# DannielSilva/MM-VQA

Hardware: AMD Instinct MI355X
Metric: samples/sec ROCO-MLM pretrain (resnet152+transformer, bs16/GPU, 224^2, seq32) (higher is better)
Workload: dtype f32; 1 GPU; pretrain/roco_train.py MLM-only: resnet152 + transformer(4 layers, 12 heads), num_vis 5, hidden 768, vocab 30522, per-GPU batch 16, 224x224, T=32; fwd + log_softmax/NLL + bwd + grad all-reduce + Adam; dropout on, train-mode BN; random-init weights; global_batch=16, seq_len=32, parallelism=dp1

## Files before the change

### mm-vqa_amd/csrc/common.h

```cpp
#pragma once
#include <hip/hip_runtime.h>
#include <stdint.h>
#include "../../include/mmvqa.h"

typedef float f32x4 __attribute__((ext_vector_type(4)));
typedef float f32x16 __attribute__((ext_vector_type(16)));

enum { ACT_NONE = 0, ACT_RELU = 1, ACT_GELU = 2, ACT_SERF = 3, ACT_SILU = 4, ACT_SIGMOID = 5 };
enum { PRO_NONE = 0, PRO_AFFINE_RELU = 1, PRO_DZ = 2, PRO_AFFINE = 3, PRO_AFFINE_SILU = 4, PRO_SILU_GATE = 5 };
enum { EPI_PLAIN = 0, EPI_TAP_FWD = 1, EPI_TAP_BWD = 2 };
enum { KIND_FWD = 0, KIND_DGRAD = 1, KIND_WGRAD = 2 };


typedef mmvqa_gemm_desc GemmParams;
typedef mmvqa_attn_desc AttnParams;

__device__ __forceinline__ float erf_pos(float s) {
  float t = 1.0f + s * (0.0705230784f + s * (0.0422820123f + s * (0.0092705272f +
            s * (0.0001520143f + s * (0.0002765672f + s * 0.0000430638f)))));
  t = t * t; t = t * t; t = t * t; t = t * t;
  const float big = 1.0f - 1.0f / t;
  const float s2 = s * s;
  float pl = -7.5757575757e-4f;
  pl = pl * s2 + 4.6296296296e-3f;
// ... 51 lines not shown
  }
}

__device__ __forceinline__ float rng_uniform(uint32_t seed, uint32_t idx) {
  uint32_t x = idx * 0x9E3779B1u + seed;
  x ^= x >> 16; x *= 0x7feb352du;
  x ^= x >> 15; x *= 0x846ca68bu;
  x ^= x >> 16;
  x += seed * 0x85ebca6bu;
  x ^= x >> 13; x *= 0xc2b2ae35u;
  x ^= x >> 16;
  return (float)(x >> 8) * (1.0f / 16777216.0f);
}

__device__ __forceinline__ float wave_sum(float v) {
#pragma unroll
  for (int o = 32; o > 0; o >>= 1) v += __shfl_xor(v, o, 64);
  return v;
}
__device__ __forceinline__ float wave_max(float v) {
#pragma unroll
  for (int o = 32; o > 0; o >>= 1) v = fmaxf(v, __shfl_xor(v, o, 64));
  return v;
}
__device__ __forceinline__ double wave_sum_d(double v) {
#pragma unroll
  for (int o = 32; o > 0; o >>= 1) v += __shfl_xor(v, o, 64);
  return v;
}

typedef mmvqa_bn_fold BnFold;
typedef double f64x2 __attribute__((ext_vector_type(2)));

__device__ __forceinline__ void bn_fold_sums(const double* __restrict__ stat, int slots, int C, int c, double& s0,
                                             double& s1) {
  f64x2 v[MMVQA_STAT_SLOTS];
#pragma unroll
  for (int k = 0; k < MMVQA_STAT_SLOTS; ++k) {
    v[k] = f64x2{0.0, 0.0};
    if (k < slots) v[k] = *reinterpret_cast<const f64x2*>(stat + ((size_t)k * C + c) * 2);
  }
  s0 = 0.0; s1 = 0.0;
#pragma unroll
  for (int k = 0; k < MMVQA_STAT_SLOTS; ++k) { s0 += v[k][0]; s1 += v[k][1]; }
}

__device__ __forceinline__ void bn_fold_fwd(const BnFold& f, int C, int c, bool pub, float& scale, float& shift) {
  double s, ss;
  bn_fold_sums(f.stat, f.slots, C, c, s, ss);
  const double mu = s / f.count;
  double var = ss / f.count - mu * mu;
  if (var < 0.0) var = 0.0;
  const float mean = (float)mu;
  const float invstd = (float)(1.0 / sqrt(var + (double)f.eps));
  scale = f.gamma[c] * invstd;
  shift = f.beta[c] - mean * scale;
  if (pub) {
    f.out0[c] = scale; f.out1[c] = shift; f.out2[c] = mean; f.out3[c] = invstd;
    if (f.run_mean) {
      const double unb = f.count > 1.0 ? var * (f.count / (f.count - 1.0)) : var;
      f.run_mean[c] = (float)(f.keep * (double)f.run_mean[c] + (1.0 - f.keep) * mu);
      f.run_var[c] = (float)(f.keep * (double)f.run_var[c] + (1.0 - f.keep) * unb);
    }
  }
}

template <int NCH>
__device__ __forceinline__ void bn_coef_block_fwd(const float* __restrict__ s, const float* __restrict__ b, const BnFold& f,
                                                  int C, int c0, bool pub, float (*cf)[NCH]) {
  const int t = threadIdx.x;
  if (t < NCH) {
    float a = 0.f, d = 0.f;
    const int c = c0 + t;
    if (c < C) {
      if (f.stat) bn_fold_fwd(f, C, c, pub, a, d);
      else { a = s[c]; d = b[c]; }
    }
    cf[0][t] = a; cf[1][t] = d;
  }
  __syncthreads();
}

__device__ __forceinline__ void bn_fold_bwd(const BnFold& f, int C, int c, bool pub, float& P, float& Q, float& R) {
  double sg, sgx;
  bn_fold_sums(f.stat, f.slots, C, c, sg, sgx);
  const double is = (double)f.invstd[c];
  const double p = (double)f.gamma[c] * is;
  const double c1 = sg / f.count, c2 = sgx / f.count;
  P = (float)p;
  Q = (float)(-p * c2 * is);
  R = (float)(p * (c2 * is * (double)f.mean[c] - c1));
  if (pub) {
    f.out0[c] = P; f.out1[c] = Q; f.out2[c] = R;
    f.dgamma[c] += (float)sgx;
    f.dbeta[c] += (float)sg;
  }
}

template <int NCH>
__device__ __forceinline__ void bn_coef_block_bwd(const float* __restrict__ P, const float* __restrict__ Q,
                                                  const float* __restrict__ R, const BnFold& f, int C, int c0, bool pub,
                                                  float (*cf)[NCH]) {
  const int t = threadIdx.x;
  if (t < NCH) {
    float p = 0.f, q = 0.f, r = 0.f;
    const int c = c0 + t;
    if (c < C) {
      if (f.stat) bn_fold_bwd(f, C, c, pub, p, q, r);
      else { p = P[c]; q = Q[c]; r = R[c]; }
    }
    cf[0][t] = p; cf[1][t] = q; cf[2][t] = r;
  }
  __syncthreads();
}

int mmvqa_set_error(int code, const char* fmt, ...);
#define MMVQA_OK 0
#define MMVQA_ERR_ARG -1
#define MMVQA_ERR_HIP -2
#define MMVQA_ERR_STATE -3

#define HIP_CHECK_RET(expr)                                                               \
  do {                                                                                    \
    hipError_t _e = (expr);                                                               \
    if (_e != hipSuccess)                                                                 \
      return mmvqa_set_error(MMVQA_ERR_HIP, "%s failed: %s (%s:%d)", #expr,               \
                             hipGetErrorString(_e), __FILE__, __LINE__);                  \
  } while (0)

// ... 2 lines not shown
```

### mm-vqa_amd/csrc/igemm.hip

```cpp
#include <string>
#include <type_traits>
#include <vector>

#include "kernels.h"

struct FastDiv {
  uint32_t mul, shr, d;
};
struct GemmAux {
  FastDiv ohw, ow;
  int fast;
  int stagger;
  float* part;
  int ldsc;
  int pad0;
  int sk_gx, sk_gy;
  int sk_slots;
  float* sk_part;
  unsigned* sk_cnt;
  int tick;
  int xcd;
};

__device__ __forceinline__ int fdiv(int n, const FastDiv& f) {
// ... 41 lines not shown
#define TRACE_MARK(i)                                                                              \
  do {                                                                                             \
    if (g_igemm_trace && threadIdx.x == 0 && TRACE_WG < TRACE_CAP0) {                              \
      unsigned long long* t_ = g_igemm_trace + ((size_t)(blockIdx.z * gridDim.y + blockIdx.y) * gridDim.x + blockIdx.x) * 8; \
      t_[i] = __builtin_readcyclecounter();                                                        \
      if ((i) == 0) {                                                                              \
        t_[5] = (unsigned long long)__builtin_amdgcn_s_getreg(4 | (0 << 6) | (31 << 11)) |         \
                ((unsigned long long)__builtin_amdgcn_s_getreg(20 | (0 << 6) | (31 << 11)) << 32); \
        t_[6] = __builtin_amdgcn_s_memrealtime();                                                  \
      }                                                                                            \
      if ((i) == 4) t_[7] = __builtin_amdgcn_s_memrealtime();                                      \
    }                                                                                              \
  } while (0)
#define TRACE_STALL_DECL unsigned long long tr_vm = 0, tr_lgkm = 0, tr_bar = 0;
#define TRACE_STALL_FLUSH()                                                                        \
  do {                                                                                             \
    if (g_igemm_trace && threadIdx.x == 0 && TRACE_WG < TRACE_CAP1) {                              \
      unsigned long long* t_ = g_igemm_trace + (1 << 22) + ((size_t)(blockIdx.z * gridDim.y + blockIdx.y) * gridDim.x + blockIdx.x) * 8; \
      t_[0] = tr_vm; t_[1] = tr_lgkm; t_[2] = tr_bar;                                              \
    }                                                                                              \
  } while (0)
#define TRACE_EPI(i)                                                                               \
  do {                                                                                             \
    if (g_igemm_trace && threadIdx.x == 0 && TRACE_WG < TRACE_CAP1)                                \
      g_igemm_trace[(1 << 22) + ((size_t)(blockIdx.z * gridDim.y + blockIdx.y) * gridDim.x + blockIdx.x) * 8 + 4 + (i)] = __builtin_readcyclecounter(); \
  } while (0)
#else
#define TRACE_MARK(i) do {} while (0)
#define TRACE_EPI(i) do {} while (0)
#define TRACE_STALL_DECL
#define TRACE_STALL_FLUSH() do {} while (0)
#endif

template <int BM, int BN, int NT, class Src>
__device__ __forceinline__ void general_epilogue(const GemmParams& p, int m0, int n0, int tid, float* smem, int slot_seed, Src src) {
  constexpr int CH = BN / 4;
  constexpr int RP = NT / CH;
  constexpr int NPASS = BM / RP;
  const int M = p.M, N = p.N;
  const int c4 = tid % CH, rg = tid / CH;
  const int col = n0 + c4 * 4;
  const bool full = col + 3 < N;
  auto ldv = [&](const float* base, size_t off) __attribute__((always_inline)) {
    f32x4 r = {0, 0, 0, 0};
    if (full && !(off & 3)) r = ld4(base + off);
    else {
#pragma unroll
      for (int j = 0; j < 4; ++j) if (col + j < N) r[j] = base[off + j];
    }
    return r;
  };
  auto stv = [&](float* base, size_t off, f32x4 v) __attribute__((always_inline)) {
    if (full && !(off & 3)) *reinterpret_cast<f32x4*>(base + off) = v;
    else {
#pragma unroll
      for (int j = 0; j < 4; ++j) if (col + j < N) base[off + j] = v[j];
    }
  };
  {
    float* C = p.C; const int ldc = p.c_ld;
    float* Cpre = p.Cpre;
    const float* Pre = p.Pre; const int dact = p.dact, pre_ld = p.pre_ld, act = p.act;
    const float* R = p.R; const int r_ld = p.r_ld;
    const float* Mk = p.Mk; const int mk_ld = p.mk_ld, mk_mode = p.mk_mode;
    const float* Z1 = p.Z1; const float* Z2 = p.Z2; const int z1_ld = p.z1_ld, z2_ld = p.z2_ld;
    double* st1 = p.stat1; double* st2 = p.stat2; const int stat_bwd = p.stat_bwd;
    float* colsum = p.colsum;
    const float drop_p = p.drop_p; const uint32_t drop_seed = p.drop_seed;
    const float keep_scale = drop_p > 0.f ? 1.0f / (1.0f - drop_p) : 1.f;
    const bool cok = col < N;
    f32x4 bias = {0, 0, 0, 0}, mks = {1, 1, 1, 1}, mkb = {0, 0, 0, 0};
    f32x4 mu1 = {0, 0, 0, 0}, is1 = {0, 0, 0, 0}, mu2 = {0, 0, 0, 0}, is2 = {0, 0, 0, 0};
    if (cok) {
      if (p.bias) bias = ldv(p.bias, col);
      if (Mk && p.mk_s) { mks = ldv(p.mk_s, col); mkb = ldv(p.mk_b, col); }
      if (st1 && stat_bwd) { mu1 = ldv(p.mean1, col); is1 = ldv(p.invstd1, col); }
      if (st2) { mu2 = ldv(p.mean2, col); is2 = ldv(p.invstd2, col); }
    }
    f32x4 sa = {0, 0, 0, 0}, sb = {0, 0, 0, 0}, sc = {0, 0, 0, 0}, cs = {0, 0, 0, 0};
    TRACE_EPI(3);
    constexpr int UP = NPASS < 4 ? NPASS : 4;
#pragma unroll 1
    for (int ps0 = 0; ps0 < NPASS; ps0 += UP) {
      if (m0 + rg + ps0 * RP >= M || !cok) break;
      f32x4 vv[UP], pr[UP], rr[UP], mm[UP], zz[UP], zz2[UP];
      bool ok[UP];
#pragma unroll
      for (int u = 0; u < UP; ++u) {
        const int rl = rg + (ps0 + u) * RP, row = m0 + rl;
        ok[u] = row < M;
        const size_t rw = ok[u] ? (size_t)row : (size_t)m0;
        vv[u] = src(rl, c4);
        if (dact) pr[u] = ldv(Pre, rw * pre_ld + col);
        if (R) rr[u] = ldv(R, rw * r_ld + col);
        if (Mk) mm[u] = ldv(Mk, rw * mk_ld + col);
        if (st1 && stat_bwd) {
          zz[u] = ldv(Z1, rw * z1_ld + col);
          if (st2) zz2[u] = ldv(Z2, rw * z2_ld + col);
        }
      }
#pragma unroll
      for (int u = 0; u < UP; ++u) {
        if (!ok[u]) continue;
        const int row = m0 + rg + (ps0 + u) * RP;
        f32x4 v = vv[u] + bias;
        if (Cpre) stv(Cpre, (size_t)row * ldc + col, v);
        if (dact) {
#pragma unroll
          for (int j = 0; j < 4; ++j) v[j] *= act_bwd(dact, pr[u][j]);
        }
        if (act) {
#pragma unroll
          for (int j = 0; j < 4; ++j) v[j] = act_fwd(act, v[j]);
        }
        if (drop_p > 0.f) {
#pragma unroll
          for (int j = 0; j < 4; ++j) {
            const float uu = rng_uniform(drop_seed, (uint32_t)row * (uint32_t)N + (uint32_t)(col + j));
            v[j] = (uu >= drop_p) ? v[j] * keep_scale : 0.f;
          }
        }
        if (R) v += rr[u];
        if (Mk) {
          if (mk_mode == 0) {
#pragma unroll
            for (int j = 0; j < 4; ++j) v[j] = (mm[u][j] * mks[j] + mkb[j] > 0.f) ? v[j] : 0.f;
          } else {
#pragma unroll
            for (int j = 0; j < 4; ++j) v[j] *= dsilu_f(mm[u][j] * mks[j] + mkb[j]);
          }
        }
#ifndef EXP_NOSTOREC
        stv(C, (size_t)row * ldc + col, v);
#endif
        if (st1) {
          if (stat_bwd) {
#pragma unroll
            for (int j = 0; j < 4; ++j) { sa[j] += v[j]; sb[j] += v[j] * ((zz[u][j] - mu1[j]) * is1[j]); }
            if (st2) {
#pragma unroll
              for (int j = 0; j < 4; ++j) sc[j] += v[j] * ((zz2[u][j] - mu2[j]) * is2[j]);
            }
          } else {
#pragma unroll
            for (int j = 0; j < 4; ++j) { sa[j] += v[j]; sb[j] += v[j] * v[j]; }
          }
        }
        if (colsum) cs += v;
      }
    }
    TRACE_EPI(1);
    if (st1 || colsum) {
      __syncthreads();
      double* red = reinterpret_cast<double*>(smem);
      float* redf = smem + BN * 6;
      for (int i = tid; i < BN * 3; i += NT) red[i] = 0.0;
      for (int i = tid; i < BN; i += NT) redf[i] = 0.f;
      __syncthreads();
      if (cok) {
        if (st1) {
#pragma unroll
          for (int j = 0; j < 4; ++j) {
            double* d = red + (c4 * 4 + j) * 3;
            atomicAdd(d, (double)sa[j]);
            atomicAdd(d + 1, (double)sb[j]);
            if (st2) atomicAdd(d + 2, (double)sc[j]);
          }
        }
        if (colsum) {
#pragma unroll
          for (int j = 0; j < 4; ++j) atomicAdd(&redf[c4 * 4 + j], cs[j]);
        }
      }
      __syncthreads();
      TRACE_EPI(2);
      if (tid < BN && n0 + tid < N) {
        if (st1) {
          const double* d = red + tid * 3;
          const int slot = slot_seed & ((p.stat_slots > 0 ? p.stat_slots : MMVQA_STAT_SLOTS) - 1);
          double* d1 = st1 + ((size_t)slot * N + n0 + tid) * 2;
          atomicAdd(d1, d[0]);
// ... 56 lines not shown
      by = (int)(r % gy);
      bz = (int)(r / gy);
    } else {
      by = (int)(Lg % gy);
      const unsigned r = Lg / gy;
      bx = (int)(r % gx);
      bz = (int)(r / gx);
    }
  }
  const int m0 = by * BM, n0 = bx * BN;
#ifdef EXP_SAMETILE
  const int lm0 = 0, ln0 = 0;
#else
  const int lm0 = m0, ln0 = n0;
#endif

  const int kt_begin = bz * p.ktiles_per_split;
  int kt_end = kt_begin + p.ktiles_per_split;
  if (kt_end > nkt_total) kt_end = nkt_total;
  const int nkt = kt_end - kt_begin;
  const int k_begin = kt_begin * BK;

  const int OHW = p.g_OH * p.g_OW;
  const int taps = p.g_KH * p.g_KW;
  const int s = p.g_stride;

  if (!NCHW && A_ROWK && tid < MAX_TAPS) {
    int t = tid < taps ? tid : 0;
    int kh = t / p.g_KW, kw = t - kh * p.g_KW;
    int off = (KIND == KIND_FWD) ? (kh * p.g_SW + kw) * p.a_ld : -((kh / s) * p.g_SW + (kw / s)) * p.a_ld;
    taptab[tid] = off;
  }
  const int fold_C = A_ROWK ? p.g_Cs : BM;
  if (x.ldsc) {
    const BnFold& f = p.a_fold;
    const bool pub = f.publish && bx == 0 && by == 0 && bz == 0;
    if constexpr (A_ROWK) {
      for (int c = tid; c < fold_C; c += NT) {
        float k0, k1, k2 = 0.f;
        if (f.bwd) bn_fold_bwd(f, fold_C, c, pub, k0, k1, k2); else bn_fold_fwd(f, fold_C, c, pub, k0, k1);
        ctab[c] = k0; ctab[fold_C + c] = k1;
        if (f.bwd) ctab[2 * fold_C + c] = k2;
      }
      if (pub && tid == 0 && !f.bwd && f.nbt) *f.nbt += f.reps;
    } else {
      if (tid < BM) {
        const int c = lm0 + tid;
        float k0 = 1.f, k1 = 0.f, k2 = 0.f;
        if (c < p.M) { if (f.bwd) bn_fold_bwd(f, p.M, c, false, k0, k1, k2); else bn_fold_fwd(f, p.M, c, false, k0, k1); }
        ctab[tid] = k0; ctab[BM + tid] = k1; ctab[2 * BM + tid] = k2;
      }
    }
  }
  __syncthreads();

  const int a_kq = (tid % KQ) * 4;
  const int a_r0 = tid / KQ;
  int a_base[NAC];
  uint32_t a_mask[NAC];
  int a_c = 0, a_tap = 0;
  int a_pix[NAC], a_y0[NAC], a_x0[NAC];
  int a_img[NAC];
  f32x4 ac0_i = {1, 1, 1, 1}, ac1_i = {0, 0, 0, 0}, ac2_i = {0, 0, 0, 0};
  const int akm_x4 = tid % A_X4, akm_k0 = tid / A_X4;
  if constexpr (A_ROWK) {
    if (x.fast == 0) {
      int k = k_begin + a_kq;
      if (taps > 1) { a_tap = k / p.g_Cs; a_c = k - a_tap * p.g_Cs; } else { a_c = k; a_tap = (k >= p.g_Cs) ? 1 : 0; }
    }
#pragma unroll
    for (int r = 0; r < NA; ++r) {
      const int row = lm0 + a_r0 + RSTEP * r;
      a_base[r] = 0; a_mask[r] = 0; a_pix[r] = 0; a_y0[r] = -(1 << 24); a_x0[r] = -(1 << 24); a_img[r] = 0;
      if (row < p.M) {
        const int n = fdiv(row, x.ohw), rem = row - n * OHW;
        const int oy = fdiv(rem, x.ow), ox = rem - oy * p.g_OW;
        if (p.gate_hw > 0) a_img[r] = row / p.gate_hw;
        if constexpr (NCHW) {
          a_pix[r] = n; a_y0[r] = oy * s - p.g_pad; a_x0[r] = ox * s - p.g_pad;
        } else if (KIND == KIND_FWD) {
          const int y0 = oy * s - p.g_pad, x0 = ox * s - p.g_pad;
          a_base[r] = ((n * p.g_SH + y0) * p.g_SW + x0) * p.a_ld;
          uint32_t xb = 0;
          for (int kw = 0; kw < p.g_KW; ++kw) xb |= ((unsigned)(x0 + kw) < (unsigned)p.g_SW ? 1u : 0u) << kw;
          uint32_t mk = 0;
          for (int kh = 0; kh < p.g_KH; ++kh) mk |= ((unsigned)(y0 + kh) < (unsigned)p.g_SH ? xb : 0u) << (kh * p.g_KW);
// ... 2 lines not shown
          const int ty = oy + p.g_pad, tx = ox + p.g_pad;
          if (s <= 2) {
            const int sh = s - 1, sm = s - 1;
            const int qy = ty >> sh, ry = ty & sm, qx = tx >> sh, rx = tx & sm;
            a_base[r] = ((n * p.g_SH + qy) * p.g_SW + qx) * p.a_ld;
            uint32_t xb = 0;
            for (int kw = 0; kw < p.g_KW; ++kw)
              xb |= (((kw & sm) == rx && (unsigned)(qx - (kw >> sh)) < (unsigned)p.g_SW) ? 1u : 0u) << kw;
            uint32_t mk = 0;
            for (int kh = 0; kh < p.g_KH; ++kh)
              mk |= (((kh & sm) == ry && (unsigned)(qy - (kh >> sh)) < (unsigned)p.g_SH) ? xb : 0u) << (kh * p.g_KW);
            a_mask[r] = mk;
          } else {
            const int qy = ty / s, ry = ty - qy * s, qx = tx / s, rx = tx - qx * s;
            a_base[r] = ((n * p.g_SH + qy) * p.g_SW + qx) * p.a_ld;
            uint32_t mk = 0;
            for (int t = 0; t < taps; ++t) {
              const int kh = t / p.g_KW, kw = t - kh * p.g_KW;
              const int sy = qy - kh / s, sx = qx - kw / s;
              if ((kh % s) == ry && (kw % s) == rx && sy >= 0 && sy < p.g_SH && sx >= 0 && sx < p.g_SW) mk |= 1u << t;
            }
            a_mask[r] = mk;
          }
        }
      }
    }
  } else {
    const int i = lm0 + akm_x4 * 4;
#pragma unroll
    for (int r = 0; r < NA_KM; ++r) {
      a_base[r] = (k_begin + akm_k0 + A_KSTEP * r) * p.a_ld + i;
      a_mask[r] = (i < p.M) ? 1u : 0u;
    }
    if (p.a_pro != PRO_NONE && i < p.M) {
      if (x.ldsc) {
        ac0_i = *reinterpret_cast<const f32x4*>(&ctab[akm_x4 * 4]);
        ac1_i = *reinterpret_cast<const f32x4*>(&ctab[BM + akm_x4 * 4]);
        ac2_i = *reinterpret_cast<const f32x4*>(&ctab[2 * BM + akm_x4 * 4]);
      } else {
        ac0_i = ld4(p.a_c0 + i); ac1_i = ld4(p.a_c1 + i);
        if (p.a_pro == PRO_DZ) ac2_i = ld4(p.a_c2 + i);
      }
    }
  }

  const int b_kq = (tid % KQ) * 4, b_r0 = tid / KQ;
  const int bkm_x4 = tid % B_X4, bkm_k0 = tid / B_X4;
  int b_base[NBC];
  uint32_t b_ok0[NBC];
  int b_co[NBC], b_tap[NBC];
  f32x4 bc0 = {1, 1, 1, 1}, bc1 = {0, 0, 0, 0};
  int b_kh = 0, b_kw = 0, b_ci = 0;
  int b_dy[4], b_dx[4], b_cc[4];
  bool b_colvalid = true;
  if constexpr (KIND == KIND_FWD) {
#pragma unroll
    for (int r = 0; r < NB; ++r) {
      const int n = ln0 + b_r0 + RSTEP * r;
      b_ok0[r] = n < p.N;
      b_base[r] = (n < p.N ? n : 0) * p.b_ld + b_kq + k_begin;
    }
  } else if constexpr (KIND == KIND_DGRAD) {
    const int n = ln0 + bkm_x4 * 4;
    b_colvalid = n < p.N;
#pragma unroll
    for (int r = 0; r < NB_KM; ++r) {
      int k = k_begin + bkm_k0 + B_KSTEP * r;
      b_tap[r] = 0; b_co[r] = k;
      if (x.fast == 0) {
        if (taps > 1) { b_tap[r] = k / p.g_Cs; b_co[r] = k - b_tap[r] * p.g_Cs; }
        else { b_tap[r] = (k >= p.g_Cs) ? 1 : 0; }
      }
      b_base[r] = n; b_ok0[r] = 1;
    }
  } else {
// ... 9 lines not shown
      for (int j = 0; j < 4; ++j) {
        int kk = nn + j;
        int tap = kk / p.g_Cs;
        b_cc[j] = kk - tap * p.g_Cs;
        b_dy[j] = tap / p.g_KW; b_dx[j] = tap - b_dy[j] * p.g_KW;
        if (kk >= p.N) b_dy[j] = -(1 << 24);
      }
    }
#pragma unroll
    for (int r = 0; r < NB_KM; ++r) { b_base[r] = k_begin + bkm_k0 + B_KSTEP * r; b_ok0[r] = 1; }
  }

  struct Stage {
    f32x4 ra[NAC], ra2[NAC], rb[NBC], rb2[NBC];
    uint32_t a_ok, b_ok;
    f32x4 ac0, ac1, ac2;
    int tm[NAC];
    int pm[NBC], tmb[NBC];
  };

  f32x16 acc[TM][TN];
#pragma unroll
  for (int i = 0; i < TM; ++i)
#pragma unroll
    for (int j = 0; j < TN; ++j)
#pragma unroll
      for (int e = 0; e < 16; ++e) acc[i][j][e] = 0.f;

  const int adv_tap = BK / p.g_Cs, adv_c = BK - adv_tap * p.g_Cs;

  auto lds_put = [&](float* tile, int e, f32x4 v) __attribute__((always_inline)) {
    if constexpr (F16) *reinterpret_cast<f16x4*>(reinterpret_cast<_Float16*>(tile) + e) = __builtin_convertvector(v, f16x4);
    else *reinterpret_cast<f32x4*>(&tile[e]) = v;
  };

  auto run = [&](auto APRO_T, auto BPRO_T, auto FAST_T, auto LDSC_T) __attribute__((always_inline)) {
    constexpr int APRO = decltype(APRO_T)::value;
    constexpr int BPRO = decltype(BPRO_T)::value;
    constexpr int FAST = decltype(FAST_T)::value;
    constexpr bool LDSC = decltype(LDSC_T)::value;
    constexpr bool A_TWO = (APRO == PRO_DZ);
    constexpr bool A_AFF = (APRO == PRO_AFFINE_RELU || APRO == PRO_AFFINE_SILU || APRO == PRO_SILU_GATE);
    constexpr bool B_AFF = (BPRO == PRO_AFFINE_RELU || BPRO == PRO_AFFINE_SILU || BPRO == PRO_SILU_GATE);

    constexpr int NLP = 1 + NAC + NBC;
    bool lt_kvalid = false;
    int lt_toff = 0;
    int lt_kh[4], lt_kw[4], lt_c[4];
    auto load_piece = [&](Stage& S, int kt, int i) __attribute__((always_inline)) {
      if (i == 0) {
        S.a_ok = 0; S.b_ok = 0;
        if constexpr (A_ROWK && !NCHW) {
          lt_kvalid = a_tap < taps;
          lt_toff = taptab[lt_kvalid ? a_tap : 0];
          if constexpr (A_AFF || A_TWO) {
            const int cc = lt_kvalid ? a_c : 0;
            S.ac0 = ld4(p.a_c0 + cc); S.ac1 = ld4(p.a_c1 + cc);
            if constexpr (APRO == PRO_DZ) S.ac2 = ld4(p.a_c2 + cc);
          }
        }
        if constexpr (NCHW) {
          S.a_ok = S.b_ok = ~0u;
          if constexpr (A_ROWK) {
#pragma unroll
            for (int j = 0; j < 4; ++j) {
              const int kk = kt * BK + a_kq + j;
// ... 192 lines not shown
        rB = __builtin_amdgcn_make_buffer_rsrc((void*)p.B, 0, p.N * p.b_ld * 4, FLAGS);
#pragma unroll
        for (int r = 0; r < NBC; ++r) f_voffB[r] = b_ok0[r] ? b_base[r] * 4 : BIG;
      } else if constexpr (KIND == KIND_DGRAD) {
        rB = __builtin_amdgcn_make_buffer_rsrc((void*)p.B, 0, p.g_Cs * p.b_ld * 4, FLAGS);
#pragma unroll
        for (int r = 0; r < NBC; ++r)
          f_voffB[r] = b_colvalid ? ((bkm_k0 + B_KSTEP * r) * p.b_ld + b_base[r]) * 4 : BIG;
      } else if constexpr (FAST == 1) {
        rB = __builtin_amdgcn_make_buffer_rsrc((void*)p.B, 0, p.K * p.b_ld * 4, FLAGS);
#pragma unroll
        for (int r = 0; r < NBC; ++r) f_voffB[r] = b_colvalid ? (b_base[r] * p.b_ld + b_ci) * 4 : BIG;
      } else {
        f_tapw = n0 / p.g_Cs;
        const int kh = f_tapw / p.g_KW, kw = f_tapw - kh * p.g_KW;
        rB = __builtin_amdgcn_make_buffer_rsrc((void*)(p.B - (p.g_pad * p.g_SW + p.g_pad) * p.b_ld), 0, NREC, FLAGS);
        rT = __builtin_amdgcn_make_buffer_rsrc((void*)p.pixmask, 0, p.K * 4, FLAGS);
        f_runB = (kh * p.g_SW + kw) * p.b_ld * 4;
#pragma unroll
        for (int r = 0; r < NBC; ++r) {
          f_voffB[r] = b_colvalid ? (b_base[r] * p.b_ld + b_ci) * 4 : BIG;
          f_voffT[r] = b_base[r] * 4;
        }
      }
#pragma unroll
      for (int r = 0; r < NBC; ++r) f_veB[r] = f_voffB[r];
    }
    int f_ve[NAC];
#pragma unroll
    for (int r = 0; r < NAC; ++r) f_ve[r] = (FAST != 0) ? f_voffA[r] : 0;
    auto tload = [&](int voff, int soff) __attribute__((always_inline)) {
      return __builtin_amdgcn_raw_buffer_load_b32(rT, voff, soff, 0);
    };
    auto f_halo = [&](Stage& S) __attribute__((always_inline)) {
      if constexpr (FAST == 2 && KIND == KIND_WGRAD) {
#pragma unroll
        for (int r = 0; r < NBC; ++r) {
          const int t = __builtin_amdgcn_sbfe(S.pm[r], f_tapw, 1);
          S.tmb[r] = t;
          f_veB[r] = (t & f_voffB[r]) | (~t & BIG);
          S.pm[r] = tload(f_voffT[r], f_runT + 2 * BK * 4);
        }
      } else if constexpr (FAST == 2) {
#pragma unroll
        for (int r = 0; r < NAC; ++r) {
          const int t = __builtin_amdgcn_sbfe((int)a_mask[r], f_tap & 31, 1);
          S.tm[r] = t;
          f_ve[r] = (t & f_voffA[r]) | (~t & BIG);
        }
      }
    };
    auto f_scalars = [&](Stage& S) __attribute__((always_inline)) {
      if constexpr (A_ROWK) {
        const bool live = f_tap < taps;
        const int toff = (KIND == KIND_FWD) ? (f_kh * p.g_SW + f_kw) * p.a_ld
                                            : f_maxneg - ((f_kh >> f_sh) * p.g_SW + (f_kw >> f_sh)) * p.a_ld;
        f_sA = live ? (toff + f_c) * 4 : BIG;
        f_sC = live ? f_c * 4 : BIG;
        if constexpr (KIND == KIND_DGRAD) f_sB = live ? (f_c * p.b_ld + f_tap * p.b_tapstride) * 4 : BIG;
        else f_sB = f_runB;
        if constexpr ((A_AFF || A_TWO) && LDSC) {
          const float* cp = ctab + f_c + a_kq;
          S.ac0 = *reinterpret_cast<const f32x4*>(cp); S.ac1 = *reinterpret_cast<const f32x4*>(cp + fold_C);
          if constexpr (APRO == PRO_DZ) S.ac2 = *reinterpret_cast<const f32x4*>(cp + 2 * fold_C);
        } else if constexpr (A_AFF || A_TWO) {
          S.ac0 = bload(rC0, f_voffC, f_sC); S.ac1 = bload(rC1, f_voffC, f_sC);
          if constexpr (APRO == PRO_DZ) S.ac2 = bload(rC2, f_voffC, f_sC);
        }
      } else {
        f_sA = f_runA; f_sB = f_runB;
      }
    };
    auto f_chunk = [&](Stage& S, int i) __attribute__((always_inline)) {
      if (i < NAC) {
        S.ra[i] = bload(rA, f_ve[i], f_sA);
        if constexpr (A_TWO) S.ra2[i] = bload(rA2, f_ve[i], f_sA);
      } else {
        S.rb[i - NAC] = bload(rB, f_veB[i - NAC], f_sB);
      }
    };
    auto f_advance = [&]() __attribute__((always_inline)) {
#ifdef EXP_NOADVANCE
      return;
#endif
      if constexpr (A_ROWK) {
        f_c += BK;
        if (f_c >= p.g_Cs) {
          f_c = 0; ++f_tap; ++f_kw;
          if (f_kw == p.g_KW) { f_kw = 0; ++f_kh; }
        }
        f_runB += BK * 4;
      } else {
        f_runA += BK * p.a_ld * 4;
        f_runB += BK * p.b_ld * 4;
        f_runT += BK * 4;
      }
    };
    auto fload_piece = [&](Stage& S, int i) __attribute__((always_inline)) {
      if (i == 0) { f_halo(S); f_scalars(S); }
      else f_chunk(S, i - 1);
      if (i == NLP - 1) f_advance();
    };
    auto fstore_chunk = [&](Stage& S, int buf, int c) __attribute__((always_inline)) {
      float* as = As + buf * A_TILE;
      float* bs = Bs + buf * B_TILE;
// ... 27 lines not shown
        } else {
          lds_put(as, (akm_k0 + A_KSTEP * r) * LDA_KM + akm_x4 * 4, v);
        }
      } else {
        const int r = c - NAC;
        f32x4 v = S.rb[r];
        if constexpr (KIND == KIND_WGRAD && BPRO == PRO_AFFINE_RELU) {
          const f32x2 lo = __builtin_elementwise_fma(v.xy, bc0.xy, bc1.xy), hi = __builtin_elementwise_fma(v.zw, bc0.zw, bc1.zw);
          if constexpr (FAST == 2) {
            const float lim = __builtin_bit_cast(float, S.tmb[r] & 0x7f800000);
            v[0] = __builtin_amdgcn_fmed3f(lo[0], 0.f, lim); v[1] = __builtin_amdgcn_fmed3f(lo[1], 0.f, lim);
            v[2] = __builtin_amdgcn_fmed3f(hi[0], 0.f, lim); v[3] = __builtin_amdgcn_fmed3f(hi[1], 0.f, lim);
          } else {
            v[0] = fmaxf(lo[0], 0.f); v[1] = fmaxf(lo[1], 0.f); v[2] = fmaxf(hi[0], 0.f); v[3] = fmaxf(hi[1], 0.f);
          }
        }
        if constexpr (B_ROWK) {
          lds_put(bs, (b_r0 + RSTEP * r) * LDK + b_kq, v);
        } else {
          lds_put(bs, (bkm_k0 + B_KSTEP * r) * LDB_KM + bkm_x4 * 4, v);
        }
      }
    };
    auto LP = [&](Stage& S, int kt, int i) __attribute__((always_inline)) {
      if constexpr (FAST != 0) fload_piece(S, i); else load_piece(S, kt, i);
    };
    auto SC = [&](Stage& S, int buf, int kt, int c) __attribute__((always_inline)) {
      if constexpr (FAST != 0) fstore_chunk(S, buf, c); else store_chunk(S, buf, kt, c);
    };
    auto LT = [&](Stage& S, int kt) __attribute__((always_inline)) {
#pragma unroll
      for (int i = 0; i < NLP; ++i) LP(S, kt, i);
    };

    auto read_frags = [&](const float* as, const float* bs, int kg, f32x4 (&fa)[TM], f32x4 (&fb)[TN]) __attribute__((always_inline)) {
#pragma unroll
      for (int i = 0; i < TM; ++i) {
        if constexpr (A_ROWK) {
          fa[i] = *reinterpret_cast<const f32x4*>(&as[(wm0 + i * 32 + li) * LDK + kg * 8 + lh * 4]);
        } else {
#pragma unroll
          for (int j = 0; j < 4; ++j) fa[i][j] = as[(kg * 8 + lh * 4 + j) * LDA_KM + wm0 + i * 32 + li];
        }
      }
#pragma unroll
      for (int i = 0; i < TN; ++i) {
        if constexpr (B_ROWK) {
          fb[i] = *reinterpret_cast<const f32x4*>(&bs[(wn0 + i * 32 + li) * LDK + kg * 8 + lh * 4]);
        } else {
#pragma unroll
          for (int j = 0; j < 4; ++j) fb[i][j] = bs[(kg * 8 + lh * 4 + j) * LDB_KM + wn0 + i * 32 + li];
        }
      }
    };

    constexpr int NC = NAC + NBC;
    constexpr int NKG = BK / 8 / KS;

    TRACE_MARK(1);
    Stage S0, S1;
    S0.a_ok = S0.b_ok = S1.a_ok = S1.b_ok = 0;
    S0.ac0 = S1.ac0 = ac0_i; S0.ac1 = S1.ac1 = ac1_i; S0.ac2 = S1.ac2 = ac2_i;

    if constexpr (FAST == 2 && KIND == KIND_WGRAD) {
#pragma unroll
      for (int r = 0; r < NBC; ++r) { S0.pm[r] = tload(f_voffT[r], 0); S1.pm[r] = tload(f_voffT[r], BK * 4); }
    }
    if (nkt > 0) {
      LT(S0, kt_begin);
      if constexpr (PIPE) LT(S1, kt_begin + 1);
#pragma unroll
      for (int c = 0; c < NC; ++c) SC(S0, 0, kt_begin, c);
      if constexpr (FAST != 0 && PIPE && !F16) f_halo(S0);
    }
    __builtin_amdgcn_s_waitcnt(0x0F70);
    __syncthreads();
    TRACE_MARK(2);

    if constexpr (F16) {
      auto frag = [&](const float* tile, int rowk, int ldkm, int r0, int st) __attribute__((always_inline)) {
        const _Float16* t = reinterpret_cast<const _Float16*>(tile);
        if (rowk) return *reinterpret_cast<const f16x8*>(t + (r0 + li) * LDK + st * 16 + lh * 8);
        const int g = lane >> 4, q = (lane >> 2) & 3, pp = lane & 3;
        const _Float16* b = t + (st * 16 + (g >> 1) * 8 + q) * ldkm + r0 + (g & 1) * 16 + 4 * pp;
        typedef __attribute__((address_space(3))) s16x4 lds_s16x4;
        const f16x4 lo = __builtin_bit_cast(f16x4, __builtin_amdgcn_ds_read_tr16_b64_v4i16((lds_s16x4*)(b)));
        const f16x4 hi = __builtin_bit_cast(f16x4, __builtin_amdgcn_ds_read_tr16_b64_v4i16((lds_s16x4*)(b + 4 * ldkm)));
        return __builtin_shufflevector(lo, hi, 0, 1, 2, 3, 4, 5, 6, 7);
      };
      auto body16 = [&](int t, Stage& Sload, Stage& Sstore) __attribute__((always_inline)) {
        const int buf = t & 1;
        LT(Sload, kt_begin + t + (PIPE ? 2 : 1));
        const float* as = As + buf * A_TILE;
        const float* bs = Bs + buf * B_TILE;
#pragma unroll
        for (int st = 0; st < BK / 16; ++st) {
          f16x8 fa[TM], fb[TN];
#pragma unroll
          for (int i = 0; i < TM; ++i) fa[i] = frag(as, A_ROWK, LDA_KM, wm0 + i * 32, st);
#pragma unroll
          for (int i = 0; i < TN; ++i) fb[i] = frag(bs, B_ROWK, LDB_KM, wn0 + i * 32, st);
#pragma unroll
          for (int a = 0; a < TM; ++a)
// ... 188 lines not shown
      } else if (x.fast == 2) {
        if constexpr (TM * TN == 1) {
          if (p.a_pro == PRO_DZ) {
            if (p.b_pro == PRO_AFFINE_RELU) run(I2{}, I1{}, F2{}, L0{}); else run(I2{}, I0{}, F2{}, L0{});
          } else {
            if (p.b_pro == PRO_AFFINE_RELU) run(I0{}, I1{}, F2{}, L0{}); else run(I0{}, I0{}, F2{}, L0{});
          }
        }
      } else if (p.a_pro == PRO_DZ) {
        switch (p.b_pro) {
          case PRO_AFFINE_RELU: run(I2{}, I1{}, G{}, L0{}); break;
          case PRO_AFFINE_SILU: run(I2{}, I4{}, G{}, L0{}); break;
          case PRO_SILU_GATE: run(I2{}, I5{}, G{}, L0{}); break;
          default: run(I2{}, I0{}, G{}, L0{});
        }
      } else {
        switch (p.b_pro) {
          case PRO_AFFINE_RELU: run(I0{}, I1{}, G{}, L0{}); break;
          case PRO_AFFINE_SILU: run(I0{}, I4{}, G{}, L0{}); break;
          case PRO_SILU_GATE: run(I0{}, I5{}, G{}, L0{}); break;
          default: run(I0{}, I0{}, G{}, L0{});
        }
      }
    }
  }

  TRACE_MARK(3);
  TRACE_STALL_FLUSH();
  constexpr int LDC = BN + 4;
  constexpr int CH = BN / 4;
  constexpr int RP = NT / CH;
  constexpr int NPASS = BM / RP;
  float* ctile = smem;
  if (KS == 1 || ks == 0) {
    static_for<TM * TN * 16>([&](auto I) {
      constexpr int i = decltype(I)::value;
      constexpr int a = i / (TN * 16), b = (i / 16) % TN, e = i % 16;
      ctile[(wm0 + a * 32 + (e & 3) + 8 * (e >> 2) + 4 * lh) * LDC + wn0 + b * 32 + li] = acc[a][b][e];
    });
  }
  __syncthreads();
  if constexpr (KS > 1) {
    if (ks == 1) {
      static_for<TM * TN * 16>([&](auto I) {
        constexpr int i = decltype(I)::value;
        constexpr int a = i / (TN * 16), b = (i / 16) % TN, e = i % 16;
        ctile[(wm0 + a * 32 + (e & 3) + 8 * (e >> 2) + 4 * lh) * LDC + wn0 + b * 32 + li] += acc[a][b][e];
      });
    }
    __syncthreads();
  }

  TRACE_EPI(0);
  const int M = p.M, N = p.N;
  const int c4 = tid % CH, rg = tid / CH;
  const int col = n0 + c4 * 4;
  const bool full = col + 3 < N;
  auto ldv = [&](const float* base, size_t off) __attribute__((always_inline)) {
    f32x4 r = {0, 0, 0, 0};
    if (full && !(off & 3)) r = ld4(base + off);
    else {
#pragma unroll
      for (int j = 0; j < 4; ++j) if (col + j < N) r[j] = base[off + j];
    }
    return r;
  };
  auto stv = [&](float* base, size_t off, f32x4 v) __attribute__((always_inline)) {
    if (full && !(off & 3)) *reinterpret_cast<f32x4*>(base + off) = v;
    else {
#pragma unroll
      for (int j = 0; j < 4; ++j) if (col + j < N) base[off + j] = v[j];
    }
  };

  if (x.tick != 0) {
    const int n_contrib = x.sk_slots, my = bz, tile_id = by * x.sk_gx + bx;
    constexpr int Q = BM * BN / 4;
    __amdgpu_buffer_rsrc_t rP = __builtin_amdgcn_make_buffer_rsrc((void*)(x.sk_part + (size_t)tile_id * x.sk_slots * (BM * BN)), 0,
                                                                  x.sk_slots * BM * BN * 4, 0x00020000);
    typedef int i32x4 __attribute__((ext_vector_type(4)));
    for (int i = tid; i < Q; i += NT) {
      const int r = i / (BN / 4), c = i - r * (BN / 4);
      const f32x4 v = *reinterpret_cast<const f32x4*>(&ctile[r * LDC + c * 4]);
      __builtin_amdgcn_raw_buffer_store_b128(__builtin_bit_cast(i32x4, v), rP, (my * Q + i) * 16, 0, SC1_AUX);
    }
    asm volatile("s_waitcnt vmcnt(0)" ::: "memory");
// ... 85 lines not shown
    }
    flush();
    __syncthreads();
    for (int i = tid; i < NIMG * BN; i += NT) {
      const int sl = i / BN, cl = i - sl * BN;
      const float v = lacc[i];
      if (v != 0.f && n0 + cl < N) atomicAdd(&out[(size_t)(img0 + sl) * N + n0 + cl], v);
    }
    TRACE_MARK(4);
    return;
  }

  if (p.epi_mode == EPI_TAP_BWD) {
    const int act = p.act, HW = p.tap_HW, ldc = p.c_ld;
    const float inv_hw = 1.0f / (float)HW;
    const float* dv = p.tap_dv;
    float* C = p.C;
#pragma unroll 1
    for (int ps = 0; ps < NPASS; ++ps) {
      const int rl = rg + ps * RP, row = m0 + rl;
      if (row >= M || col >= N) break;
      const int img = row / HW;
      f32x4 v = *reinterpret_cast<const f32x4*>(&ctile[rl * LDC + c4 * 4]);
      const f32x4 g = ldv(dv, (size_t)img * N + col);
#pragma unroll
      for (int j = 0; j < 4; ++j) v[j] = g[j] * inv_hw * act_bwd(act, v[j]);
      stv(C, (size_t)row * ldc + col, v);
    }
    TRACE_MARK(4);
    return;
  }

  general_epilogue<BM, BN, NT>(p, m0, n0, tid, smem, (int)(blockIdx.y + blockIdx.x * 7 + blockIdx.z * 3),
                               [&](int rl, int cq) __attribute__((always_inline)) {
                                 return *reinterpret_cast<const f32x4*>(&ctile[rl * LDC + cq * 4]);
                               });
  TRACE_MARK(4);
}

constexpr int FOLD_MAX_FLOATS = 3072;
constexpr int SK_MAX = 8;

__global__ __launch_bounds__(256) void splitk_finish_kernel(const GemmParams p, const float* __restrict__ part,
                                                            int nsplit) {
  constexpr int BM = 64, BN = 64;
  __shared__ double smem_d[BN * 3 + BN / 2 + 2];
  const int tid = threadIdx.x, m0 = blockIdx.y * BM, n0 = blockIdx.x * BN;
  const int M = p.M, N = p.N;
  const size_t MN = (size_t)M * N;
  general_epilogue<BM, BN, 256>(p, m0, n0, tid, reinterpret_cast<float*>(smem_d), (int)(blockIdx.y + blockIdx.x * 7),
                                [&](int rl, int cq) __attribute__((always_inline)) {
                                  f32x4 v = {0, 0, 0, 0};
                                  const int row = m0 + rl, col = n0 + cq * 4;
                                  if (row < M && col < N) {
                                    const size_t off = (size_t)row * N + col;
                                    if (col + 3 < N && !(off & 3)) {
                                      f32x4 t[SK_MAX];
#pragma unroll
                                      for (int s = 0; s < SK_MAX; ++s)
                                        t[s] = s < nsplit ? ld4(part + s * MN + off) : f32x4{0, 0, 0, 0};
#pragma unroll
                                      for (int s = 0; s < SK_MAX; ++s) v += t[s];
                                    } else {
                                      for (int s = 0; s < nsplit; ++s)
#pragma unroll
                                        for (int j = 0; j < 4; ++j)
                                          if (col + j < N) v[j] += part[s * MN + off + j];
                                    }
                                  }
                                  return v;
                                });
}

static FastDiv make_fastdiv(int d) {
  FastDiv f;
  f.d = (uint32_t)d;
  if (d <= 1) { f.mul = 0; f.shr = 0; f.d = 1; return f; }
  int lg = 31;
  while (lg > 0 && !((uint32_t)d >> lg)) --lg;
  if (d & (d - 1)) ++lg;
  const int pw = 31 + lg;
  const uint64_t m = ((1ull << pw) + (uint64_t)d - 1) / (uint64_t)d;
  f.mul = (uint32_t)m;
// ... 329 lines not shown
```

Measured before the change: 662.8 samples/s.

## Overlap BN-fold stat loads and epilogue side loads with GEMM prologue and staging

The BN fold coefficient computation now issues its stat and parameter loads early (bn_fold_issue) and finishes the table only after the first A/B tile loads are in flight, so that global-load latency overlaps. In the plain epilogue, side-tensor loads (residual, pre-activation, mask, BN inputs) are issued before the accumulator is staged to shared memory, hiding their latency behind the LDS writes and barrier. The stat fold loop is also changed from a fixed full-slot unroll to grouped loads of four slots with a runtime loop, and the per-element stat accumulation is vectorized. This adds control complexity and register pressure in the GEMM prologue and epilogue.

```diff
diff --git a/mm-vqa_amd/csrc/common.h b/mm-vqa_amd/csrc/common.h
--- a/mm-vqa_amd/csrc/common.h
+++ b/mm-vqa_amd/csrc/common.h
@@ -107,29 +107,57 @@
 typedef mmvqa_bn_fold BnFold;
 typedef double f64x2 __attribute__((ext_vector_type(2)));
 
+#define BN_FOLD_GROUP 4
+__device__ __forceinline__ void bn_fold_group(const double* __restrict__ stat, int slots, int C, int c, int k0,
+                                              f64x2 (&v)[BN_FOLD_GROUP]) {
+#pragma unroll
+  for (int j = 0; j < BN_FOLD_GROUP; ++j) {
+    v[j] = f64x2{0.0, 0.0};
+    if (k0 + j < slots) v[j] = *reinterpret_cast<const f64x2*>(stat + ((size_t)(k0 + j) * C + c) * 2);
+  }
+}
+__device__ __forceinline__ void bn_fold_sums_from(const double* __restrict__ stat, int slots, int C, int c,
+                                                  const f64x2 (&v0)[BN_FOLD_GROUP], double& s0, double& s1) {
+  s0 = 0.0; s1 = 0.0;
+#pragma unroll
+  for (int j = 0; j < BN_FOLD_GROUP; ++j) { s0 += v0[j][0]; s1 += v0[j][1]; }
+#pragma unroll 1
+  for (int k0 = BN_FOLD_GROUP; k0 < slots; k0 += BN_FOLD_GROUP) {
+    f64x2 v[BN_FOLD_GROUP];
+    bn_fold_group(stat, slots, C, c, k0, v);
+#pragma unroll
+    for (int j = 0; j < BN_FOLD_GROUP; ++j) { s0 += v[j][0]; s1 += v[j][1]; }
+  }
+}
 __device__ __forceinline__ void bn_fold_sums(const double* __restrict__ stat, int slots, int C, int c, double& s0,
                                              double& s1) {
-  f64x2 v[MMVQA_STAT_SLOTS];
-#pragma unroll
-  for (int k = 0; k < MMVQA_STAT_SLOTS; ++k) {
-    v[k] = f64x2{0.0, 0.0};
-    if (k < slots) v[k] = *reinterpret_cast<const f64x2*>(stat + ((size_t)k * C + c) * 2);
-  }
-  s0 = 0.0; s1 = 0.0;
-#pragma unroll
-  for (int k = 0; k < MMVQA_STAT_SLOTS; ++k) { s0 += v[k][0]; s1 += v[k][1]; }
-}
-
-__device__ __forceinline__ void bn_fold_fwd(const BnFold& f, int C, int c, bool pub, float& scale, float& shift) {
+  f64x2 v0[BN_FOLD_GROUP];
+  bn_fold_group(stat, slots, C, c, 0, v0);
+  bn_fold_sums_from(stat, slots, C, c, v0, s0, s1);
+}
+
+struct BnFoldIn {
+  f64x2 v0[BN_FOLD_GROUP];
+  float g, b, m;
+};
+__device__ __forceinline__ void bn_fold_issue(const BnFold& f, bool bwd, int C, int c, BnFoldIn& in) {
+  bn_fold_group(f.stat, f.slots, C, c, 0, in.v0);
+  const float* pb = bwd ? f.invstd : f.beta;
+  const float* pm = bwd ? f.mean : f.gamma;
+  in.g = f.gamma[c]; in.b = pb[c]; in.m = pm[c];
+}
+
+__device__ __forceinline__ void bn_fold_fwd_from(const BnFold& f, int C, int c, bool pub, const BnFoldIn& in, float& scale,
+                                                 float& shift) {
   double s, ss;
-  bn_fold_sums(f.stat, f.slots, C, c, s, ss);
+  bn_fold_sums_from(f.stat, f.slots, C, c, in.v0, s, ss);
   const double mu = s / f.count;
   double var = ss / f.count - mu * mu;
   if (var < 0.0) var = 0.0;
   const float mean = (float)mu;
   const float invstd = (float)(1.0 / sqrt(var + (double)f.eps));
-  scale = f.gamma[c] * invstd;
-  shift = f.beta[c] - mean * scale;
+  scale = in.g * invstd;
+  shift = in.b - mean * scale;
   if (pub) {
     f.out0[c] = scale; f.out1[c] = shift; f.out2[c] = mean; f.out3[c] = invstd;
     if (f.run_mean) {
@@ -138,6 +166,11 @@
       f.run_var[c] = (float)(f.keep * (double)f.run_var[c] + (1.0 - f.keep) * unb);
     }
   }
+}
+__device__ __forceinline__ void bn_fold_fwd(const BnFold& f, int C, int c, bool pub, float& scale, float& shift) {
+  BnFoldIn in;
+  bn_fold_issue(f, false, C, c, in);
+  bn_fold_fwd_from(f, C, c, pub, in, scale, shift);
 }
 
 template <int NCH>
@@ -156,20 +189,26 @@
   __syncthreads();
 }
 
-__device__ __forceinline__ void bn_fold_bwd(const BnFold& f, int C, int c, bool pub, float& P, float& Q, float& R) {
+__device__ __forceinline__ void bn_fold_bwd_from(const BnFold& f, int C, int c, bool pub, const BnFoldIn& in, float& P,
+                                                 float& Q, float& R) {
   double sg, sgx;
-  bn_fold_sums(f.stat, f.slots, C, c, sg, sgx);
-  const double is = (double)f.invstd[c];
-  const double p = (double)f.gamma[c] * is;
+  bn_fold_sums_from(f.stat, f.slots, C, c, in.v0, sg, sgx);
+  const double is = (double)in.b;
+  const double p = (double)in.g * is;
   const double c1 = sg / f.count, c2 = sgx / f.count;
   P = (float)p;
   Q = (float)(-p * c2 * is);
-  R = (float)(p * (c2 * is * (double)f.mean[c] - c1));
+  R = (float)(p * (c2 * is * (double)in.m - c1));
   if (pub) {
     f.out0[c] = P; f.out1[c] = Q; f.out2[c] = R;
     f.dgamma[c] += (float)sgx;
     f.dbeta[c] += (float)sg;
   }
+}
+__device__ __forceinline__ void bn_fold_bwd(const BnFold& f, int C, int c, bool pub, float& P, float& Q, float& R) {
+  BnFoldIn in;
+  bn_fold_issue(f, true, C, c, in);
+  bn_fold_bwd_from(f, C, c, pub, in, P, Q, R);
 }
 
 template <int NCH>
diff --git a/mm-vqa_amd/csrc/igemm.hip b/mm-vqa_amd/csrc/igemm.hip
--- a/mm-vqa_amd/csrc/igemm.hip
+++ b/mm-vqa_amd/csrc/igemm.hip
@@ -97,8 +97,8 @@
 #define TRACE_STALL_FLUSH() do {} while (0)
 #endif
 
-template <int BM, int BN, int NT, class Src>
-__device__ __forceinline__ void general_epilogue(const GemmParams& p, int m0, int n0, int tid, float* smem, int slot_seed, Src src) {
+template <int BM, int BN, int NT, class Stage, class Src>
+__device__ __forceinline__ void general_epilogue(const GemmParams& p, int m0, int n0, int tid, float* smem, int slot_seed, Stage stage, Src src) {
   constexpr int CH = BN / 4;
   constexpr int RP = NT / CH;
   constexpr int NPASS = BM / RP;
@@ -143,19 +143,15 @@
       if (st2) { mu2 = ldv(p.mean2, col); is2 = ldv(p.invstd2, col); }
     }
     f32x4 sa = {0, 0, 0, 0}, sb = {0, 0, 0, 0}, sc = {0, 0, 0, 0}, cs = {0, 0, 0, 0};
-    TRACE_EPI(3);
     constexpr int UP = NPASS < 4 ? NPASS : 4;
-#pragma unroll 1
-    for (int ps0 = 0; ps0 < NPASS; ps0 += UP) {
-      if (m0 + rg + ps0 * RP >= M || !cok) break;
-      f32x4 vv[UP], pr[UP], rr[UP], mm[UP], zz[UP], zz2[UP];
-      bool ok[UP];
+    f32x4 pr[UP], rr[UP], mm[UP], zz[UP], zz2[UP];
+    bool ok[UP];
+    auto side_loads = [&](int ps0) __attribute__((always_inline)) {
 #pragma unroll
       for (int u = 0; u < UP; ++u) {
-        const int rl = rg + (ps0 + u) * RP, row = m0 + rl;
+        const int row = m0 + rg + (ps0 + u) * RP;
         ok[u] = row < M;
         const size_t rw = ok[u] ? (size_t)row : (size_t)m0;
-        vv[u] = src(rl, c4);
         if (dact) pr[u] = ldv(Pre, rw * pre_ld + col);
         if (R) rr[u] = ldv(R, rw * r_ld + col);
         if (Mk) mm[u] = ldv(Mk, rw * mk_ld + col);
@@ -164,6 +160,11 @@
           if (st2) zz2[u] = ldv(Z2, rw * z2_ld + col);
         }
       }
+    };
+    auto passes = [&](int ps0) __attribute__((always_inline)) {
+      f32x4 vv[UP];
+#pragma unroll
+      for (int u = 0; u < UP; ++u) vv[u] = src(rg + (ps0 + u) * RP, c4);
 #pragma unroll
       for (int u = 0; u < UP; ++u) {
         if (!ok[u]) continue;
@@ -199,19 +200,28 @@
         stv(C, (size_t)row * ldc + col, v);
 #endif
         if (st1) {
+          sa += v;
           if (stat_bwd) {
-#pragma unroll
-            for (int j = 0; j < 4; ++j) { sa[j] += v[j]; sb[j] += v[j] * ((zz[u][j] - mu1[j]) * is1[j]); }
-            if (st2) {
-#pragma unroll
-              for (int j = 0; j < 4; ++j) sc[j] += v[j] * ((zz2[u][j] - mu2[j]) * is2[j]);
-            }
+            sb += v * ((zz[u] - mu1) * is1);
+            if (st2) sc += v * ((zz2[u] - mu2) * is2);
           } else {
-#pragma unroll
-            for (int j = 0; j < 4; ++j) { sa[j] += v[j]; sb[j] += v[j] * v[j]; }
+            sb += v * v;
           }
         }
         if (colsum) cs += v;
+      }
+    };
+    const bool rows0 = cok && m0 + rg < M;
+    if (rows0) side_loads(0);
+    stage();
+    TRACE_EPI(3);
+    if (rows0) {
+      passes(0);
+#pragma unroll 1
+      for (int ps0 = UP; ps0 < NPASS; ps0 += UP) {
+        if (m0 + rg + ps0 * RP >= M) break;
+        side_loads(ps0);
+        passes(ps0);
       }
     }
     TRACE_EPI(1);
@@ -334,26 +344,9 @@
     taptab[tid] = off;
   }
   const int fold_C = A_ROWK ? p.g_Cs : BM;
-  if (x.ldsc) {
-    const BnFold& f = p.a_fold;
-    const bool pub = f.publish && bx == 0 && by == 0 && bz == 0;
-    if constexpr (A_ROWK) {
-      for (int c = tid; c < fold_C; c += NT) {
-        float k0, k1, k2 = 0.f;
-        if (f.bwd) bn_fold_bwd(f, fold_C, c, pub, k0, k1, k2); else bn_fold_fwd(f, fold_C, c, pub, k0, k1);
-        ctab[c] = k0; ctab[fold_C + c] = k1;
-        if (f.bwd) ctab[2 * fold_C + c] = k2;
-      }
-      if (pub && tid == 0 && !f.bwd && f.nbt) *f.nbt += f.reps;
-    } else {
-      if (tid < BM) {
-        const int c = lm0 + tid;
-        float k0 = 1.f, k1 = 0.f, k2 = 0.f;
-        if (c < p.M) { if (f.bwd) bn_fold_bwd(f, p.M, c, false, k0, k1, k2); else bn_fold_fwd(f, p.M, c, false, k0, k1); }
-        ctab[tid] = k0; ctab[BM + tid] = k1; ctab[2 * BM + tid] = k2;
-      }
-    }
-  }
+  const int fold_N = A_ROWK ? p.g_Cs : p.M;
+  const int fold_c = A_ROWK ? tid : lm0 + (tid & (BM - 1));
+  BnFoldIn fold_in;
   __syncthreads();
 
   const int a_kq = (tid % KQ) * 4;
@@ -422,15 +415,9 @@
       a_base[r] = (k_begin + akm_k0 + A_KSTEP * r) * p.a_ld + i;
       a_mask[r] = (i < p.M) ? 1u : 0u;
     }
-    if (p.a_pro != PRO_NONE && i < p.M) {
-      if (x.ldsc) {
-        ac0_i = *reinterpret_cast<const f32x4*>(&ctab[akm_x4 * 4]);
-        ac1_i = *reinterpret_cast<const f32x4*>(&ctab[BM + akm_x4 * 4]);
-        ac2_i = *reinterpret_cast<const f32x4*>(&ctab[2 * BM + akm_x4 * 4]);
-      } else {
-        ac0_i = ld4(p.a_c0 + i); ac1_i = ld4(p.a_c1 + i);
-        if (p.a_pro == PRO_DZ) ac2_i = ld4(p.a_c2 + i);
-      }
+    if (p.a_pro != PRO_NONE && i < p.M && !x.ldsc) {
+      ac0_i = ld4(p.a_c0 + i); ac1_i = ld4(p.a_c1 + i);
+      if (p.a_pro == PRO_DZ) ac2_i = ld4(p.a_c2 + i);
     }
   }
 
@@ -506,6 +493,32 @@
   auto lds_put = [&](float* tile, int e, f32x4 v) __attribute__((always_inline)) {
     if constexpr (F16) *reinterpret_cast<f16x4*>(reinterpret_cast<_Float16*>(tile) + e) = __builtin_convertvector(v, f16x4);
     else *reinterpret_cast<f32x4*>(&tile[e]) = v;
+  };
+
+  auto fold_table = [&]() __attribute__((always_inline)) {
+    const BnFold& f = p.a_fold;
+    if constexpr (A_ROWK) {
+      const bool pub = f.publish && bx == 0 && by == 0 && bz == 0;
+      if (tid < fold_C) {
+        float k0, k1, k2 = 0.f;
+        if (f.bwd) bn_fold_bwd_from(f, fold_C, tid, pub, fold_in, k0, k1, k2); else bn_fold_fwd_from(f, fold_C, tid, pub, fold_in, k0, k1);
+        ctab[tid] = k0; ctab[fold_C + tid] = k1;
+        if (f.bwd) ctab[2 * fold_C + tid] = k2;
+      }
+      for (int c = tid + NT; c < fold_C; c += NT) {
+        float k0, k1, k2 = 0.f;
+        if (f.bwd) bn_fold_bwd(f, fold_C, c, pub, k0, k1, k2); else bn_fold_fwd(f, fold_C, c, pub, k0, k1);
+        ctab[c] = k0; ctab[fold_C + c] = k1;
+        if (f.bwd) ctab[2 * fold_C + c] = k2;
+      }
+      if (pub && tid == 0 && !f.bwd && f.nbt) *f.nbt += f.reps;
+    } else {
+      if (tid < BM) {
+        float k0 = 1.f, k1 = 0.f, k2 = 0.f;
+        if (fold_c < p.M) { if (f.bwd) bn_fold_bwd_from(f, p.M, fold_c, false, fold_in, k0, k1, k2); else bn_fold_fwd_from(f, p.M, fold_c, false, fold_in, k0, k1); }
+        ctab[tid] = k0; ctab[BM + tid] = k1; ctab[2 * BM + tid] = k2;
+      }
+    }
   };
 
   auto run = [&](auto APRO_T, auto BPRO_T, auto FAST_T, auto LDSC_T) __attribute__((always_inline)) {
@@ -764,6 +777,11 @@
     auto tload = [&](int voff, int soff) __attribute__((always_inline)) {
       return __builtin_amdgcn_raw_buffer_load_b32(rT, voff, soff, 0);
     };
+    auto take_coef = [&](Stage& S, int c) __attribute__((always_inline)) {
+      const float* cp = ctab + c + a_kq;
+      S.ac0 = *reinterpret_cast<const f32x4*>(cp); S.ac1 = *reinterpret_cast<const f32x4*>(cp + fold_C);
+      if constexpr (APRO == PRO_DZ) S.ac2 = *reinterpret_cast<const f32x4*>(cp + 2 * fold_C);
+    };
     auto f_halo = [&](Stage& S) __attribute__((always_inline)) {
       if constexpr (FAST == 2 && KIND == KIND_WGRAD) {
 #pragma unroll
@@ -782,7 +800,8 @@
         }
       }
     };
-    auto f_scalars = [&](Stage& S) __attribute__((always_inline)) {
+    auto f_scalars_impl = [&](Stage& S, auto COEF_T) __attribute__((always_inline)) {
+      constexpr bool COEF = decltype(COEF_T)::value;
       if constexpr (A_ROWK) {
         const bool live = f_tap < taps;
         const int toff = (KIND == KIND_FWD) ? (f_kh * p.g_SW + f_kw) * p.a_ld
@@ -792,9 +811,7 @@
         if constexpr (KIND == KIND_DGRAD) f_sB = live ? (f_c * p.b_ld + f_tap * p.b_tapstride) * 4 : BIG;
         else f_sB = f_runB;
         if constexpr ((A_AFF || A_TWO) && LDSC) {
-          const float* cp = ctab + f_c + a_kq;
-          S.ac0 = *reinterpret_cast<const f32x4*>(cp); S.ac1 = *reinterpret_cast<const f32x4*>(cp + fold_C);
-          if constexpr (APRO == PRO_DZ) S.ac2 = *reinterpret_cast<const f32x4*>(cp + 2 * fold_C);
+          if constexpr (COEF) take_coef(S, f_c);
         } else if constexpr (A_AFF || A_TWO) {
           S.ac0 = bload(rC0, f_voffC, f_sC); S.ac1 = bload(rC1, f_voffC, f_sC);
           if constexpr (APRO == PRO_DZ) S.ac2 = bload(rC2, f_voffC, f_sC);
@@ -803,6 +820,7 @@
         f_sA = f_runA; f_sB = f_runB;
       }
     };
+    auto f_scalars = [&](Stage& S) __attribute__((always_inline)) { f_scalars_impl(S, std::true_type{}); };
     auto f_chunk = [&](Stage& S, int i) __attribute__((always_inline)) {
       if (i < NAC) {
         S.ra[i] = bload(rA, f_ve[i], f_sA);
@@ -896,6 +914,16 @@
 #pragma unroll
       for (int i = 0; i < NLP; ++i) LP(S, kt, i);
     };
+    auto LT_first = [&](Stage& S, int kt) __attribute__((always_inline)) {
+      if constexpr (FAST != 0 && LDSC) {
+        f_halo(S); f_scalars_impl(S, std::false_type{});
+#pragma unroll
+        for (int i = 0; i < NAC + NBC; ++i) f_chunk(S, i);
+        f_advance();
+      } else {
+        LT(S, kt);
+      }
+    };
 
     auto read_frags = [&](const float* as, const float* bs, int kg, f32x4 (&fa)[TM], f32x4 (&fb)[TN]) __attribute__((always_inline)) {
 #pragma unroll
@@ -930,9 +958,33 @@
 #pragma unroll
       for (int r = 0; r < NBC; ++r) { S0.pm[r] = tload(f_voffT[r], 0); S1.pm[r] = tload(f_voffT[r], BK * 4); }
     }
+    constexpr bool FOLD = LDSC || !A_ROWK;
+    if constexpr (FOLD) {
+      if (x.ldsc) bn_fold_issue(p.a_fold, p.a_fold.bwd != 0, fold_N, fold_c < fold_N ? fold_c : 0, fold_in);
+    }
+    int fc0 = 0, fc1 = 0;
     if (nkt > 0) {
-      LT(S0, kt_begin);
-      if constexpr (PIPE) LT(S1, kt_begin + 1);
+      fc0 = f_c;
+      LT_first(S0, kt_begin);
+      fc1 = f_c;
+      if constexpr (PIPE) LT_first(S1, kt_begin + 1);
+    }
+    if constexpr (FOLD) {
+      if (x.ldsc) {
+        fold_table();
+        __syncthreads();
+        if constexpr (A_ROWK) {
+          take_coef(S0, fc0);
+          if constexpr (PIPE) take_coef(S1, fc1);
+        } else if (p.a_pro != PRO_NONE && lm0 + akm_x4 * 4 < p.M) {
+          ac0_i = *reinterpret_cast<const f32x4*>(&ctab[akm_x4 * 4]);
+          ac1_i = *reinterpret_cast<const f32x4*>(&ctab[BM + akm_x4 * 4]);
+          ac2_i = *reinterpret_cast<const f32x4*>(&ctab[2 * BM + akm_x4 * 4]);
+          S0.ac0 = S1.ac0 = ac0_i; S0.ac1 = S1.ac1 = ac1_i; S0.ac2 = S1.ac2 = ac2_i;
+        }
+      }
+    }
+    if (nkt > 0) {
 #pragma unroll
       for (int c = 0; c < NC; ++c) SC(S0, 0, kt_begin, c);
       if constexpr (FAST != 0 && PIPE && !F16) f_halo(S0);
@@ -1187,26 +1239,30 @@
   constexpr int RP = NT / CH;
   constexpr int NPASS = BM / RP;
   float* ctile = smem;
-  if (KS == 1 || ks == 0) {
-    static_for<TM * TN * 16>([&](auto I) {
-      constexpr int i = decltype(I)::value;
-      constexpr int a = i / (TN * 16), b = (i / 16) % TN, e = i % 16;
-      ctile[(wm0 + a * 32 + (e & 3) + 8 * (e >> 2) + 4 * lh) * LDC + wn0 + b * 32 + li] = acc[a][b][e];
-    });
-  }
-  __syncthreads();
-  if constexpr (KS > 1) {
-    if (ks == 1) {
+  auto stage_acc = [&]() __attribute__((always_inline)) {
+    if (KS == 1 || ks == 0) {
       static_for<TM * TN * 16>([&](auto I) {
         constexpr int i = decltype(I)::value;
         constexpr int a = i / (TN * 16), b = (i / 16) % TN, e = i % 16;
-        ctile[(wm0 + a * 32 + (e & 3) + 8 * (e >> 2) + 4 * lh) * LDC + wn0 + b * 32 + li] += acc[a][b][e];
+        ctile[(wm0 + a * 32 + (e & 3) + 8 * (e >> 2) + 4 * lh) * LDC + wn0 + b * 32 + li] = acc[a][b][e];
       });
     }
     __syncthreads();
-  }
-
-  TRACE_EPI(0);
+    if constexpr (KS > 1) {
+      if (ks == 1) {
+        static_for<TM * TN * 16>([&](auto I) {
+          constexpr int i = decltype(I)::value;
+          constexpr int a = i / (TN * 16), b = (i / 16) % TN, e = i % 16;
+          ctile[(wm0 + a * 32 + (e & 3) + 8 * (e >> 2) + 4 * lh) * LDC + wn0 + b * 32 + li] += acc[a][b][e];
+        });
+      }
+      __syncthreads();
+    }
+    TRACE_EPI(0);
+  };
+  const bool epi_plain = !x.tick && !x.part && !p.c_atomic && p.epi_mode == EPI_PLAIN;
+  if (!epi_plain) stage_acc();
+
   const int M = p.M, N = p.N;
   const int c4 = tid % CH, rg = tid / CH;
   const int col = n0 + c4 * 4;
@@ -1358,6 +1414,7 @@
   }
 
   general_epilogue<BM, BN, NT>(p, m0, n0, tid, smem, (int)(blockIdx.y + blockIdx.x * 7 + blockIdx.z * 3),
+                               [&]() __attribute__((always_inline)) { if (epi_plain) stage_acc(); },
                                [&](int rl, int cq) __attribute__((always_inline)) {
                                  return *reinterpret_cast<const f32x4*>(&ctile[rl * LDC + cq * 4]);
                                });
@@ -1375,6 +1432,7 @@
   const int M = p.M, N = p.N;
   const size_t MN = (size_t)M * N;
   general_epilogue<BM, BN, 256>(p, m0, n0, tid, reinterpret_cast<float*>(smem_d), (int)(blockIdx.y + blockIdx.x * 7),
+                                []() {},
                                 [&](int rl, int cq) __attribute__((always_inline)) {
                                   f32x4 v = {0, 0, 0, 0};
                                   const int row = m0 + rl, col = n0 + cq * 4;
```

New measurement: 660.3 samples/s. Within noise of the previous version (-0.4%).
